# sergiud/SuiteSparse

Measured on AMD Instinct MI355X. Metric: GFLOP/s supernodal Cholesky factor (Common->fl / t_factorize), higher is better.
Workload: dtype f64; 1 GPU; poisson3d_200^3_geometricND_leaf4; n=8000000, nsuper=428821, parallelism=1 GPU

## Files before the change

include/cholmod_hip.h:

```cpp
#ifndef CHOLMOD_HIP_H
#define CHOLMOD_HIP_H

#include <stddef.h>
#include <stdint.h>

#ifdef __cplusplus
extern "C" {
#endif

#define CHOLMOD_HIP_OK            0
#define CHOLMOD_HIP_NOT_POSDEF    1
#define CHOLMOD_HIP_NO_DEVICE   (-1)
#define CHOLMOD_HIP_OUT_OF_MEMORY (-2)
#define CHOLMOD_HIP_TOO_LARGE   (-3)
#define CHOLMOD_HIP_INVALID     (-4)
#define CHOLMOD_HIP_GPU_PROBLEM (-5)

#define CHOLMOD_HIP_PLAN_DEFAULT   0
#define CHOLMOD_HIP_TILE128         4
#define CHOLMOD_HIP_NO_SMALL_FRONTS 16
#define CHOLMOD_HIP_NO_XCD_SWIZZLE 32
#define CHOLMOD_HIP_FIXED_OB       64
#define CHOLMOD_HIP_WIDE_OB       128
#define CHOLMOD_HIP_NO_CB_ASSIGN   2048
#define CHOLMOD_HIP_NO_FUSED_POTRF 512
#define CHOLMOD_HIP_NO_FUSED_TRSM 1024
#define CHOLMOD_HIP_NO_LEAF_PAIRS 4096
#define CHOLMOD_HIP_NO_EXCHANGE_LOOKAHEAD 256
#define CHOLMOD_HIP_CHAIN256     8192
#define CHOLMOD_HIP_PHI_TWIN    16384
#define CHOLMOD_HIP_CX_STORAGE   32768
#define CHOLMOD_HIP_FUSED_CB_EA   65536
#define CHOLMOD_HIP_PLAN_HOST_ONLY 2

typedef struct cholmod_hip_plan cholmod_hip_plan ;

int cholmod_hip_probe (void) ;

int cholmod_hip_memorysize (size_t *total_mem, size_t *available_mem) ;

int cholmod_hip_set_device (int device) ;
int cholmod_hip_device_count (int *count) ;

cholmod_hip_plan *cholmod_hip_plan_create (int64_t n, int64_t nsuper,
    const int64_t *super, const int64_t *pi, const int64_t *px,
    const int64_t *s, int flags, int *status) ;

void cholmod_hip_plan_destroy (cholmod_hip_plan *plan) ;

cholmod_hip_plan *cholmod_hip_plan_create_reach (int64_t n, int64_t nsuper,
    const int64_t *super, const int64_t *pi, const int64_t *px,
    const int64_t *s, int flags, const int64_t *reach_p, const int32_t *reach_first, int *status) ;

typedef int (*cholmod_hip_allreduce_fn) (void *dev_ptr, int64_t count_doubles,
    int group_first, int group_size, void *user) ;
cholmod_hip_plan *cholmod_hip_plan_create_dist (int64_t n, int64_t nsuper,
    const int64_t *super, const int64_t *pi, const int64_t *px,
    const int64_t *s, int flags, int rank, int world, int *status) ;
int cholmod_hip_set_allreduce (cholmod_hip_plan *plan,
    cholmod_hip_allreduce_fn fn, void *user) ;
int cholmod_hip_rccl_unique_id (void *id128) ;
int cholmod_hip_rccl_attach (cholmod_hip_plan *plan, const void *id128) ;
int cholmod_hip_rccl_detach (cholmod_hip_plan *plan) ;
int64_t cholmod_hip_debug_routing (cholmod_hip_plan *plan, int64_t cap, int64_t *pair_d, int64_t *pair_a,
    int64_t *cb_lo, int64_t *cb_hi) ;
int cholmod_hip_debug_schedule_hash (cholmod_hip_plan *plan, uint64_t *out16) ;
int64_t cholmod_hip_debug_cb_extend_add (cholmod_hip_plan *plan, int64_t cap, int64_t *out) ;
int64_t cholmod_hip_debug_fused_pair (cholmod_hip_plan *plan, int64_t pair, int64_t *desc, int32_t *inv, int32_t *rel) ;
int cholmod_hip_progress_enable (cholmod_hip_plan *plan, int enable) ;
int cholmod_hip_progress (cholmod_hip_plan *plan, int64_t *out12) ;
int64_t cholmod_hip_get_batches (cholmod_hip_plan *plan, int64_t *batch_of, int64_t *global_arena) ;
int cholmod_hip_get_partition (cholmod_hip_plan *plan, int64_t *owner) ;
int cholmod_hip_get_groups (cholmod_hip_plan *plan, int64_t *first, int64_t *size) ;
int cholmod_hip_gather_factor (cholmod_hip_plan *plan) ;

int cholmod_hip_factorize (cholmod_hip_plan *plan, const int64_t *Sp,
    const int64_t *Si, const int64_t *Snz, const double *Sx, double beta,
    int quick_return_if_not_posdef, double *Lx_host, int64_t *minor) ;

int cholmod_hip_upload_matrix (cholmod_hip_plan *plan, const int64_t *Sp,
    const int64_t *Si, const int64_t *Snz, const double *Sx) ;
int cholmod_hip_factorize_resident (cholmod_hip_plan *plan, double beta,
    int quick_return_if_not_posdef, int64_t *minor) ;

int cholmod_hip_set_value_map (cholmod_hip_plan *plan, const int64_t *src, int64_t snz,
    int64_t nvalues) ;
int cholmod_hip_values_begin (cholmod_hip_plan *plan, double **buffer, const int64_t **index,
    int64_t *count, int64_t *chunk_len) ;
int cholmod_hip_values_push_chunk (cholmod_hip_plan *plan, int64_t chunk) ;

int cholmod_hip_factorize_values_device (cholmod_hip_plan *plan, const double *dvalues, int64_t nvalues,
// ... 79 lines not shown
```

suitesparse_amd/cholmod.py:

```python
from __future__ import annotations

import ctypes as C
import os
import subprocess

import numpy as np

_HERE = os.path.dirname(os.path.abspath(__file__))
LIB_PATH = os.environ.get("CHOLMOD_AMD_LIB") or os.path.join(_HERE, "lib", "libcholmod_amd.so")
HOOKS_LIB_PATH = os.path.join(_HERE, "lib", "libcholmod_amd_testhooks.so")
CSRC = os.path.join(_HERE, "csrc")

CHOLMOD_MAXMETHODS = 9
CHOLMOD_HIP_NSTATS = 41

PATTERN, REAL, COMPLEX, ZOMPLEX = 0, 1, 2, 3
OK, NOT_INSTALLED, OUT_OF_MEMORY, TOO_LARGE, INVALID, GPU_PROBLEM = 0, -1, -2, -3, -4, -5
NOT_POSDEF = 1
NATURAL, GIVEN, POSTORDERED = 0, 1, 6
SIMPLICIAL, AUTO, SUPERNODAL = 0, 1, 2
SYS_A, SYS_LDLt, SYS_LD, SYS_DLt, SYS_L, SYS_Lt, SYS_D, SYS_P, SYS_Pt = range(9)
HIP_PLAN_HOST_ONLY = 2
HIP_WIDE_OB, HIP_NO_FUSED_POTRF, HIP_NO_FUSED_TRSM, HIP_PHI_TWIN = 128, 512, 1024, 16384
HIP_NO_SMALL_FRONTS = 16
HIP_FUSED_CB_EA = 65536
HIP_OK = 0
HIP_INVALID = -4
HIP_NO_DEVICE = -1


class Method(C.Structure):
    _fields_ = [("lnz", C.c_double), ("fl", C.c_double), ("ordering", C.c_int)]


ERRFUNC = C.CFUNCTYPE(None, C.c_int, C.c_char_p, C.c_int, C.c_char_p)
ALLREDUCE_FN = C.CFUNCTYPE(C.c_int, C.c_void_p, C.c_int64, C.c_int, C.c_int, C.c_void_p)


class Common(C.Structure):
    _fields_ = [
        ("supernodal", C.c_int), ("supernodal_switch", C.c_double),
        ("final_asis", C.c_int), ("final_super", C.c_int), ("final_ll", C.c_int),
        ("final_pack", C.c_int), ("final_monotonic", C.c_int), ("final_resymbol", C.c_int),
        ("zrelax", C.c_double * 3), ("nrelax", C.c_size_t * 3),
        ("prefer_upper", C.c_int), ("quick_return_if_not_posdef", C.c_int),
        ("print", C.c_int), ("nmethods", C.c_int), ("current", C.c_int), ("selected", C.c_int),
        ("method", Method * (CHOLMOD_MAXMETHODS + 1)),
        ("postorder", C.c_int), ("try_catch", C.c_int),
# ... 95 lines not shown
    "cholmod_l_hip_aat_values_grad_device", "cholmod_l_hip_aat_logdet_grad_device",
    "cholmod_l_hip_factor_grad_device", "cholmod_l_hip_factor_outer_grad_device", "cholmod_l_hip_factor_grad_to_host",
]
HIP_SYMBOLS = [
    "cholmod_hip_probe", "cholmod_hip_memorysize", "cholmod_hip_set_device", "cholmod_hip_device_count",
    "cholmod_hip_plan_create", "cholmod_hip_plan_destroy", "cholmod_hip_factorize",
    "cholmod_hip_plan_create_dist", "cholmod_hip_plan_create_reach", "cholmod_hip_set_allreduce", "cholmod_hip_get_partition",
    "cholmod_hip_get_groups", "cholmod_hip_get_batches", "cholmod_hip_progress_enable", "cholmod_hip_progress", "cholmod_hip_debug_schedule_hash", "cholmod_hip_diag_minmax", "cholmod_hip_values_begin", "cholmod_hip_values_push_chunk", "cholmod_hip_debug_routing",
    "cholmod_hip_gather_factor",
    "cholmod_hip_upload_matrix", "cholmod_hip_factorize_resident",
    "cholmod_hip_set_value_map",
    "cholmod_hip_factorize_values_device", "cholmod_hip_set_product_map", "cholmod_hip_download_matrix_values",
    "cholmod_hip_download_factor", "cholmod_hip_download_even_columns", "cholmod_hip_upload_factor", "cholmod_hip_solve",
    "cholmod_hip_set_perm", "cholmod_hip_solve_device", "cholmod_hip_residual_device", "cholmod_hip_refine_device",
    "cholmod_hip_get_maps", "cholmod_hip_get_stats", "cholmod_hip_set_profiling",
    "cholmod_hip_selinv_device", "cholmod_hip_selinv_gather_device", "cholmod_hip_selinv_download",
    "cholmod_hip_selinv_release", "cholmod_hip_selinv_info",
    "cholmod_hip_schur_device", "cholmod_hip_trailing_multiply_device",
    "cholmod_hip_factor_grad_device", "cholmod_hip_factor_outer_grad_device", "cholmod_hip_factor_grad_gather_device",
    "cholmod_hip_factor_grad_download", "cholmod_hip_factor_grad_release", "cholmod_hip_factor_grad_info",
    "cholmod_hip_values_grad_device", "cholmod_hip_logdet_device",
    "cholmod_hip_product_values_grad_device", "cholmod_hip_product_logdet_grad_device",
    "cholmod_hip_dense_partial_factor", "cholmod_hip_factor_checks", "cholmod_hip_factor_checks_local", "cholmod_hip_get_launch_profile", "cholmod_hip_debug_thin_cycles", "cholmod_hip_debug_launch_regions",
    "cholmod_hip_debug_cb_extend_add", "cholmod_hip_debug_fused_pair",
    "cholmod_hip_rccl_unique_id", "cholmod_hip_rccl_attach", "cholmod_hip_rccl_detach",
    "cholmod_hip_version",
]

PROBES_PATH = os.path.join(_HERE, "lib", "libcholmod_amd_probes.so")
PROBE_SYMBOLS = [
    "cholmod_hip_bench_update_kernel", "cholmod_hip_bench_update_pair", "cholmod_hip_bench_mfma_peak", "cholmod_hip_bench_mfma_peak2",
    "cholmod_hip_bench_mixed", "cholmod_hip_debug_potrf_cycles", "cholmod_hip_debug_panel_cycles",
    "cholmod_hip_debug_latency", "cholmod_hip_bench_mfma_ceiling", "cholmod_hip_probe_cu_mask", "cholmod_hip_probe_overlap", "cholmod_hip_debug_update_diff", "cholmod_hip_debug_diag_cycles", "cholmod_hip_bench_handoff",
]

_probes = None


def build(force: bool = False) -> str:
    if force:
        subprocess.check_call(["make", "-C", CSRC, "-s", "clean"])
    subprocess.check_call(["make", "-C", CSRC, "-s", "-j3"])
    return LIB_PATH


_libs = {}

# ... 129 lines not shown
    sig("cholmod_hip_factor_grad_release", C.c_int, [vp])
    sig("cholmod_hip_factor_grad_info", C.c_int, [vp, vp])
    sig("cholmod_l_hip_factor_grad_device", C.c_int, [sp, fc, vp, vp, vp, vp, cm])
    sig("cholmod_l_hip_factor_outer_grad_device", C.c_int, [sp, fc, dbl, vp, sz, vp, sz, sz, vp, vp, vp, cm])
    sig("cholmod_l_hip_factor_grad_to_host", C.c_int, [fc, vp, cm])
    sig("cholmod_hip_values_grad_device", C.c_int, [vp, C.c_int, dbl, vp, i64, vp, i64, i64, vp, i64, vp])
    sig("cholmod_hip_logdet_device", C.c_int, [vp, vp, vp])
    sig("cholmod_l_hip_values_grad_device", C.c_int, [sp, fc, dbl, vp, sz, vp, sz, sz, vp, vp, cm])
    sig("cholmod_l_hip_logdet_device", C.c_int, [fc, vp, vp, cm])
    sig("cholmod_hip_product_values_grad_device", C.c_int, [vp, C.c_int, dbl, vp, i64, vp, i64, i64, vp, vp, i64, vp])
    sig("cholmod_hip_product_logdet_grad_device", C.c_int, [vp, vp, vp, i64, vp])
    sig("cholmod_l_hip_aat_values_grad_device", C.c_int, [sp, fc, dbl, vp, sz, vp, sz, sz, vp, vp, vp, cm])
    sig("cholmod_l_hip_aat_logdet_grad_device", C.c_int, [sp, fc, vp, vp, vp, cm])
    sig("cholmod_hip_get_maps", C.c_int, [vp, vp, vp, vp])
    sig("cholmod_hip_get_stats", C.c_int, [vp, vp])
    sig("cholmod_hip_set_profiling", C.c_int, [vp, C.c_int])
    sig("cholmod_hip_dense_partial_factor", C.c_int, [vp, i64, i64, C.c_int, C.POINTER(i64)])
    sig("cholmod_hip_factor_checks", C.c_int, [vp, vp])
    sig("cholmod_hip_factor_checks_local", C.c_int, [vp, vp])
    sig("cholmod_hip_get_launch_profile", i64, [vp, i64, vp, vp, vp, vp, vp, vp])
    sig("cholmod_hip_debug_thin_cycles", C.c_int, [vp, i64, vp])
    sig("cholmod_hip_debug_launch_regions", i64, [vp, i64, i64, vp])
    sig("cholmod_hip_debug_cb_extend_add", i64, [vp, i64, vp])
    sig("cholmod_hip_debug_fused_pair", i64, [vp, i64, vp, vp, vp])
    sig("cholmod_hip_rccl_unique_id", C.c_int, [vp])
    sig("cholmod_hip_rccl_attach", C.c_int, [vp, vp])
    sig("cholmod_hip_rccl_detach", C.c_int, [vp])
    sig("cholmod_hip_version", C.c_char_p, [])
    _libs[path] = L
    return L


def probes():
    global _probes
    if _probes is not None:
        return _probes
    if not os.path.exists(PROBES_PATH):
        raise RuntimeError(f"{PROBES_PATH} is missing: build it with __graft_entry__.build()")
    L = C.CDLL(PROBES_PATH)
    vp, i64, dbl = C.c_void_p, C.c_int64, C.c_double
    for name, res, args in (
            ("cholmod_hip_bench_update_kernel", dbl, [i64, i64, i64, C.c_int, C.c_int]),
            ("cholmod_hip_bench_update_pair", dbl, [i64, i64, i64, i64, i64, C.c_int, C.c_int]),
            ("cholmod_hip_bench_mfma_peak", dbl, [C.c_int, C.c_int]),
            ("cholmod_hip_bench_mfma_peak2", dbl, [C.c_int, C.c_int, C.c_int, C.c_int]),
            ("cholmod_hip_bench_mixed", dbl, [C.c_int, C.c_int, C.c_int]),
# ... 606 lines not shown
```

suitesparse_amd/csrc/hip/engine.hip:

```cpp
#include "update_launch.hip.h"
#include "chain256_kernels.hip.h"
#include "exchange_internal.hip.h"
#include <thread>

namespace {

static void drop_product_map (cholmod_hip_plan *P)
{
    for (void *d : {(void *) P->d_pm_cp, (void *) P->d_pm_ia, (void *) P->d_pm_ib, (void *) P->d_pm_order}) if (d) (void) hipFree (d) ;
    P->d_pm_cp = P->d_pm_ia = P->d_pm_ib = nullptr ; P->d_pm_order = nullptr ;
    P->pm_set = false ; P->pm_na = 0 ;
    for (void *d : {(void *) P->d_pt_ptr, (void *) P->d_pt_c, (void *) P->d_pt_partner, (void *) P->d_pt_order, (void *) P->d_pt_gvals})
        if (d) (void) hipFree (d) ;
    P->d_pt_ptr = nullptr ; P->d_pt_c = P->d_pt_partner = P->d_pt_order = nullptr ; P->d_pt_gvals = nullptr ;
    P->pt_built = false ;
}

static void free_device (cholmod_hip_plan *P)
{
    drop_product_map (P) ;
    selinv_free (P) ;
    grad_free (P) ;
    for (hipEvent_t e : {P->fv_ev_in, P->fv_ev_out}) if (e) (void) hipEventDestroy (e) ;
    P->fv_ev_in = P->fv_ev_out = nullptr ;
// ... 1357 lines not shown

int64_t cholmod_hip_debug_fused_pair (cholmod_hip_plan *P, int64_t pair, int64_t *desc, int32_t *inv, int32_t *rel)
{
    if (!P) return CHOLMOD_HIP_INVALID ;
    const Schedule &S = P->sch ;
    const i64 np = (i64) S.ivp.size () ;
    if (pair < 0 || pair >= np || !desc) return np ;
    const InvPair &R = S.ivp [pair] ;
    i64 launch = -1 ;
    for (size_t z = 0 ; z < S.fz.size () && launch < 0 ; z++)
    {
        if (S.fz [z].front != R.parent) continue ;
        const size_t q = (size_t) (std::find (S.gfz.begin (), S.gfz.end (), (i32) z) - S.gfz.begin ()) ;
        for (size_t l = 0 ; l < S.launches.size () ; l++)
            if (S.launches [l].kind == K_UPD_W && q >= S.launches [l].goff && q < S.launches [l].goff + S.launches [l].ng) launch = (i64) l ;
    }
    const i64 d [8] = {R.parent, R.child, R.pnscol, R.pncb, R.nc, P->fr [R.child].cbp, R.mcb, launch} ;
    for (int t = 0 ; t < 8 ; t++) desc [t] = d [t] ;
    if (inv && P->d_invmap) HIPCHK (hipMemcpy (inv, P->d_invmap + R.inv, (size_t) R.pncb * sizeof (i32), hipMemcpyDeviceToHost)) ;
    if (rel && P->d_relmap) HIPCHK (hipMemcpy (rel, P->d_relmap + R.rel, (size_t) R.nc * sizeof (i32), hipMemcpyDeviceToHost)) ;
    return np ;
}

int64_t cholmod_hip_debug_launch_regions (cholmod_hip_plan *P, int64_t launch, int64_t cap, int64_t *out)
{
    if (!P || launch < 0 || launch >= (i64) P->sch.launches.size ()) return CHOLMOD_HIP_INVALID ;
    const Launch &L = P->sch.launches [launch] ;
    if (L.kind != K_UPD_W && L.kind != K_UPD_SMALL && L.kind != K_UPD_BIG && L.kind != K_UPD_PF) return 0 ;
    for (i64 q = 0 ; q < L.ng && q < cap ; q++)
    {
        const GemmGroup &G = P->sch.gg [L.goff + q] ;
        const i64 v [12] = {G.m, G.n, G.k, G.tri, G.c_in_cb, G.lda, G.ldc, G.ntiles, G.nblk, G.front, G.assign, G.swz} ;
        for (int t = 0 ; t < 12 ; t++) out [12 * q + t] = v [t] ;
    }
    return L.ng ;
}

int cholmod_hip_set_profiling (cholmod_hip_plan *P, int on)
{
    if (!P) return CHOLMOD_HIP_INVALID ;
    P->profiling = on != 0 ;
    return CHOLMOD_HIP_OK ;
}

int cholmod_hip_dense_partial_factor (double *F, int64_t nsrow, int64_t nscol, int flags,
    int64_t *info_out)
{
    if (!F || nsrow <= 0 || nscol <= 0 || nscol > nsrow) return CHOLMOD_HIP_INVALID ;
    if (!cholmod_hip_probe ()) return CHOLMOD_HIP_NO_DEVICE ;
    FrontD f ;
    memset (&f, 0, sizeof (f)) ;
    f.nscol = (i32) nscol ; f.nsrow = (i32) nsrow ; f.ncb = (i32) (nsrow - nscol) ; f.parent = -1 ;
    std::vector<FrontD> fr (1, f) ;
    Schedule S ;
// ... 58 lines not shown
```

suitesparse_amd/csrc/hip/plan.hip.h:

```cpp
#pragma once
#include "descriptors.hip.h"
#include "../../../include/cholmod_hip.h"

#include <rccl/rccl.h>

#include <algorithm>
#include <atomic>
#include <cmath>
#include <cstdio>
#include <cstdlib>
#include <cstring>
#include <map>
#include <functional>
#include <memory>
#include <new>
#include <queue>
#include <vector>
#include <atomic>
#include <chrono>

#ifdef CHOLMOD_HIP_TEST_HOOKS
#define TEST_ENV(name) getenv (name)
#else
#define TEST_ENV(name) ((const char *) nullptr)
// ... 211 lines not shown
    std::vector<SolveTask> sv_tasks ;
    std::vector<i32> sv_ptr ;
    std::vector<std::vector<i32>> sv_big ;
    SolveTask *d_sv = nullptr ;
    std::vector<InvTask> inv_tasks ;
    std::vector<i64> inv_first ;
    InvTask *d_inv_tasks = nullptr ;
    double *d_winv = nullptr ;
    bool winv_valid = false ;
    double *d_solved = nullptr ; i64 solved_cap = 0 ;
    double *d_sv_acc = nullptr ; i64 sv_acc_cap = 0 ;
    struct SbLaunch { i32 level, first, ntasks, grid ; } ;
    std::vector<SolveBlk> sb_tasks, sb_commit ;
    std::vector<SbLaunch> sb_launch, sb_commit_launch ;
    std::vector<i32> sb_lvl_ptr ;
    SolveBlk *d_sb_tasks = nullptr, *d_sb_commit = nullptr ;
    int sb_max_tasks = 0 ;
    long long *d_thin_tim = nullptr ;
    CheckTask *d_chk = nullptr ; i64 nchk = 0 ;
    double *d_chk_out = nullptr ;
    Schedule sch ;
    double exec_flops = 0 ;
    std::vector<i64> reach_p ;
    std::vector<i32> reach_first, head ;
    bool head_gather = true ;
    GatherGroup *d_xg = nullptr ; i32 *d_gmap = nullptr ;
    FuseD *d_fz = nullptr ; i32 *d_gfz = nullptr, *d_invmap = nullptr ;
    hipStream_t stream = nullptr ;
    hipStream_t stream2 = nullptr ;
    std::vector<hipEvent_t> sync_ev ;
    i64 *d_Ls = nullptr ;
    FrontD *d_fr = nullptr ;
    i32 *d_supermap = nullptr, *d_child = nullptr, *d_relmap = nullptr, *d_info = nullptr ;
    i32 *d_lvl_list = nullptr ;
    double *d_Lx = nullptr, *d_cb = nullptr ;
    ZeroGroup *d_zg = nullptr ; EaGroup *d_eg = nullptr ; PfGroup *d_pg = nullptr ;
    TrGroup *d_tg = nullptr ; GemmGroup *d_gg = nullptr ; i32 *d_sm = nullptr ;
    DgGroup *d_dg = nullptr ; RsGroup *d_rg = nullptr ; double *d_dinv = nullptr ;
    std::vector<i64> lpx ;
    i64 lx_local = 0 ;
    std::vector<i64> win_off ;
    i64 lx_fronts = 0 ;
    std::vector<i64> crel ;
    std::vector<RelPair> relpairs ;
    i64 relsize_all = 0 ;
    bool passthru = false ;
    i64 *d_crel = nullptr ; RelPair *d_relpairs = nullptr ;
// ... 45 lines not shown
    int factor_state = 0 ;
    hipEvent_t sc_ev_in = nullptr, sc_ev_out = nullptr ;
    struct Grad *gr = nullptr ;
    bool gr_index_valid = false ;
    volatile long long prog_fact = 0, prog_launch = 0, prog_xchg_enq = 0 ;
    long long *prog_dev = nullptr ;
    bool profiling = false ;
    double stats [CHOLMOD_HIP_NSTATS] = {0} ;
    double solve_seconds = 0 ;
    std::vector<float> launch_ms ;
    hipEvent_t ev0 = nullptr, ev1 = nullptr ;
    std::vector<hipEvent_t> evpool ;
} ;

static inline double *whole_factor (cholmod_hip_plan *P) { return P->world == 1 ? P->d_Lx : (P->full_valid ? P->d_Lx_full : nullptr) ; }
static inline const FrontD *whole_fronts (cholmod_hip_plan *P) { return P->world == 1 ? P->d_fr : P->d_fr_full ; }

void selinv_free (cholmod_hip_plan *P) ;
void selinv_gather_logdet_grad (cholmod_hip_plan *P, const i32 *colof, double *out, hipStream_t st) ;
void grad_free (cholmod_hip_plan *P) ;

namespace sship {

struct HeadInfo { const i32 *head ; const i64 *reach_p ; const i32 *first ; bool gather ; } ;

int build_host (cholmod_hip_plan *P) ;
void schedule_dense (const std::vector<FrontD> &fr, const i32 *ids, int nf,
    Schedule &S, int flags, const i32 *owner, const i32 *grp0, const i32 *grpn, int rank, int world,
    const char *assign_cb = nullptr, const i64 *win = nullptr, const i32 *child = nullptr, bool allow_half = false,
    const HeadInfo *heads = nullptr, const i64 *crel = nullptr, const std::vector<i64> *Ls = nullptr) ;

}
```

suitesparse_amd/csrc/hip/plan_build.hip:

```cpp
#include "plan.hip.h"

namespace sship {
namespace {

struct PlanBuilder
{
    cholmod_hip_plan *P ;
    const i64 n, nsuper ;
    int nlev = 0 ;
    std::vector<i32> cptr, call ;
    std::vector<double> wsub ;
    std::vector<i32> st_stack ;
    bool distribute = false, passthru = false, cx_storage = false ;
    int ownw = 128 ;
    std::vector<i64> cb_len_all ;
    std::vector<std::vector<i32>> rel_list ;
    std::vector<std::vector<i32>> batches ;

    explicit PlanBuilder (cholmod_hip_plan *P_) : P (P_), n (P_->n), nsuper (P_->nsuper) {}

    bool mine (i64 s) const { return P->rank >= P->grp0 [s] && P->rank < P->grp0 [s] + P->grpn [s] ; }
    template <typename F> void for_subtree (i32 root, F &&fn)
    {
        st_stack.clear () ;
// ... 617 lines not shown
    }
    void schedule_batches ()
    {
        Schedule &S = P->sch ;
        std::vector<i32> mine_ids, gen ;
        P->batch_launch0.clear () ;
        for (const auto &bt : batches)
        {
            P->batch_launch0.push_back (S.launches.size ()) ;
            mine_ids.clear () ; gen.clear () ;
            for (i32 sf : bt) if (mine (sf)) mine_ids.push_back (sf) ;
            if (mine_ids.empty ()) continue ;
            schedule_thin (mine_ids, gen) ;
            const i32 *ids = gen.data () ;
            const int nf = (int) gen.size () ;
            if (nf == 0) continue ;
            schedule_zero (ids, nf) ;
            const size_t ea0 = S.launches.size (), fz0 = S.fz.size (), ivp0 = S.ivp.size () ;
            schedule_extend_add (ids, nf, 0) ;
            const bool has_ea0 = S.launches.size () > ea0 ;
            schedule_dense (P->fr, ids, nf, S, P->flags, P->owner.data (), P->grp0.data (), P->grpn.data (),
                P->rank, P->world, P->assign_cb.data (), P->win_off.data (), P->child.data (),
                P->world == 1 && !P->force_shared,
                P->head.empty () ? nullptr : &heads, P->crel.data (), &P->Ls) ;
            if (S.fz.size () == fz0) { schedule_extend_add (ids, nf, 1) ; continue ; }
            std::vector<char> fused (nf, 0) ;
            {
                std::map<i32, int> at ;
                for (int q = 0 ; q < nf ; q++) at [ids [q]] = q ;
                for (size_t z = fz0 ; z < S.fz.size () ; z++) fused [at [S.fz [z].front]] = 1 ;
            }
            if (has_ea0)
                for (size_t z = ivp0 ; z < S.ivp.size () ; z++)
                    S.launches [ea0].bytes -= 24.0 * ((double) S.ivp [z].mcb * (S.ivp [z].mcb + 1) / 2) ;
            schedule_extend_add (ids, nf, 1, &fused) ;
        }
    }

    HeadInfo heads {nullptr, nullptr, nullptr, true} ;
    void choose_heads ()
    {
        P->head.clear () ;
        if (P->reach_p.empty () || P->world != 1 || P->force_shared || getenv ("CHOLMOD_HIP_NO_HEADS")) return ;
        if (P->flags & (CHOLMOD_HIP_PHI_TWIN | CHOLMOD_HIP_CX_STORAGE | CHOLMOD_HIP_TILE128)) return ;
        const ObThresholds obt = outer_block_thresholds () ;
        const bool all = getenv ("CHOLMOD_HIP_HEAD_ALL") && atoi (getenv ("CHOLMOD_HIP_HEAD_ALL")) != 0 ;
        auto rate = [] (int K) { return 1e12 * (K < 512 ? 60.0 : K < 1024 ? 70.0 : K < 2048 ? 74.5 : 75.0) ; } ;
        auto tri = [] (double m) { return m * (m + 1) / 2 ; } ;
        std::vector<i32> head (P->nsuper, 0) ;
        bool any = false ;
        for (i64 s = 0 ; s < P->nsuper ; s++)
        {
            const FrontD &f = P->fr [s] ;
            if (P->reach_p [s + 1] - P->reach_p [s] != f.nsrow || P->owner [s] < 0) continue ;
            const i32 *first = P->reach_first.data () + P->reach_p [s] ;
            const int OB = front_ob (f, P->flags, obt) ;
            double best = all ? 0.0 : 0.25e-3 ;
            for (int H = 256 ; H < std::min (OB, (int) f.nscol) ; H += 256)
            {
                i64 R = 0 ;
                for (int p = H ; p < f.nsrow ; p++) R += first [p] < H ;
                const double N = f.nsrow - H ;
                const double gain = all ? 2.0 * H * (tri (N) - tri ((double) R))
                    : 2.0 * H * tri (N) / rate (OB) - 2.0 * H * tri ((double) R) / rate (H) - 16.0 * tri (N) / 4e12 ;
                if (gain > best) { best = gain ; head [s] = H ; any = true ; }
            }
        }
        if (!any) return ;
        P->head.swap (head) ;
        P->head_gather = !getenv ("CHOLMOD_HIP_HEAD_NO_GATHER") ;
        heads = HeadInfo {P->head.data (), P->reach_p.data (), P->reach_first.data (), P->head_gather} ;
    }

    int run ()
    {
        int rc = init_fronts () ;
        if (rc != CHOLMOD_HIP_OK) return rc ;
        rc = build_etree () ;
        if (rc != CHOLMOD_HIP_OK) return rc ;
        assign_ownership () ;
        choose_heads () ;
        layout_local_factor () ;
        build_child_lists () ;
        choose_batches () ;
        rc = build_solve_tasks () ;
        if (rc != CHOLMOD_HIP_OK) return rc ;
        layout_windows () ;
        schedule_batches () ;
        for (const Launch &L : P->sch.launches) P->stats [40] += L.skipped ;
        return CHOLMOD_HIP_OK ;
    }
} ;

}
// ... 9 lines not shown
```

suitesparse_amd/csrc/hip/schedule_dense.hip:

```cpp
#include "plan.hip.h"

namespace sship {
namespace {

struct Upd { int q, kc, kk, t0, t1 ; bool cb, wide ; } ;

struct DenseScheduler
{
    const std::vector<FrontD> &fr ;
    const i32 *ids ; const int nf ;
    Schedule &S ;
    const int flags ;
    const i32 *owner, *grp0, *grpn ;
    const int rank, world ;
    const char *assign_cb ;
    const i64 *win ;
    const i32 *child ;
    const bool allow_half ;
    const HeadInfo *heads ;
    const i64 *crel ;
    const std::vector<i64> *Ls ;
    bool cx, twin, use_big ;
    ObThresholds obt ;
    int maxnscol = 0, maxrows = 0 ;
// ... 40 lines not shown
        by_launch = true ;
        { const char *e = getenv ("CHOLMOD_HIP_UPD3_HALF_MAX") ; w_half_max = e ? (i64) atoll (e) : (i64) 10240 ; }
        w_half_min = 512 ; w_min_k = 256 ; unfuse_tiles = w_min_tiles ;
        if (!allow_half || w_min_tiles <= 0) w_half_max = 0 ;
        if (w_half_max <= 0 || w_half_min > w_min_tiles) w_half_min = w_min_tiles ;
        one_region = false ;
        swz16 = false ;
        xla = !(flags & CHOLMOD_HIP_NO_EXCHANGE_LOOKAHEAD) ;
        balance_cb = !use_big && !getenv ("CHOLMOD_HIP_NO_CB_BALANCE") ;
        early.assign (nf, -1) ; early_open.assign (nf, -1) ; pf_done.assign (nf, -1) ;
        fuse_ea = (flags & CHOLMOD_HIP_FUSED_CB_EA) && world == 1 && allow_half && !twin && !use_big && w_min_tiles > 0
            && assign_cb && child && crel && Ls ;
        choose_chain () ;
    }

    i64 co (int c, i64 ld) const { return cx ? (i64) (c >> 1) * ld : (i64) c * ld ; }
    void twin_operands (GemmGroup &G, int origin, int kc) const
    {
        if ((origin | kc | G.k | G.m | G.n | G.lda | G.ldc) & 1) { fprintf (stderr, "cholmod_hip: twin plan with an odd region\n") ; abort () ; }
        if (!cx) G.lda *= 2 ;
        G.k /= 2 ;
    }
    int ob_of (const FrontD &f) const { return front_ob (f, flags, obt) ; }
    int head_of (int fid) const { return heads && heads->head ? heads->head [fid] : 0 ; }
    void ob_bounds (int q, int i0, int &o0, int &o1) const
    {
        const FrontD &f = fr [ids [q]] ;
        const int OBq = ob_of (f), H = head_of (ids [q]) ;
        if (H > 0 && i0 < H) o0 = 0 ;
        else if (H > 0) o0 = H + ((i0 - H) / OBq) * OBq ;
        else o0 = (i0 / OBq) * OBq ;
        o1 = std::min (o0 + (H > 0 && i0 < H ? H : OBq), (int) f.nscol) ;
    }
    bool is_shared (int fid) const { return owner && owner [fid] < 0 ; }
    bool windowed (int fid) const { return win && win [fid] >= 0 ; }
    i64 psx_at (int fid, int col) const
    {
        const FrontD &f = fr [fid] ;
        if (!windowed (fid)) return f.psx ;
        int OBq = ob_of (f), ob = col / OBq ;
        return win [fid] + (i64) (ob & 1) * window_len (f, OBq) - (i64) ob * OBq * f.nsrow ;
    }
    static i64 region_tiles (const GemmGroup &G)
    {
        i64 mt = (G.m + SMALL - 1) / SMALL, nt = (G.n + SMALL - 1) / SMALL ;
        return G.tri ? nt * (nt + 1) / 2 + (mt - nt) * nt : mt * nt ;
    }
    static i64 tri_tiles (int rows, int cols)
    {
        i64 mt = (rows + SMALL - 1) / SMALL, nt = (cols + SMALL - 1) / SMALL ;
        return nt * (nt + 1) / 2 + (mt - nt) * nt ;
    }
    XchgD xchg_of (int q, int c0) const
    {
        const FrontD &f = fr [ids [q]] ;
// ... 232 lines not shown
    void flush_updates ()
    {
        if (w_min_tiles > 0 && !use_big)
        {
            i64 pooled = 0 ;
            if (by_launch) for (auto &G : small) if (G.k >= w_min_k || region_tiles (G) >= w_min_tiles) pooled += region_tiles (G) ;
            std::vector<GemmGroup> keep ;
            for (auto &G : small)
            {
                const bool w = region_tiles (G) >= w_min_tiles || (by_launch && pooled >= w_half_min && G.k >= w_min_k) ;
                if (w) wav.push_back (G) ; else keep.push_back (G) ;
            }
            small.swap (keep) ;
        }
        flush_kind (big, K_UPD_BIG) ;
        flush_kind (small, K_UPD_SMALL) ;
        flush_kind (pfv, K_UPD_PF) ;
        flush_kind (wav, K_UPD_W) ;
        flush_gathered () ;
        carrier.clear () ;
    }
    void add_head_gathered (const Upd &x)
    {
        const int fid = ids [x.q], H = x.kk ;
        const FrontD &f = fr [fid] ;
        const i32 *first = heads->first + heads->reach_p [fid] ;
        auto tri_elems = [] (double m, double n) { return n * (n + 1) / 2 + (m - n) * n ; } ;
        double full = tri_elems (f.nsrow - H, f.nscol - H) + tri_elems (f.ncb, f.ncb), done = 0 ;
        auto gathered = [&] (int from, int ncols, bool to_cb)
        {
            const size_t m0 = S.gmap.size () ;
            int n = 0 ;
            for (int p = from ; p < f.nsrow ; p += 2)
            {
                if (first [p] >= H && (p + 1 >= f.nsrow || first [p + 1] >= H)) continue ;
                S.gmap.push_back (p) ; n += p < from + ncols ;
                if (p + 1 < f.nsrow) { S.gmap.push_back (p + 1) ; n += p + 1 < from + ncols ; }
            }
            const int m = (int) (S.gmap.size () - m0) ;
            if (n == 0) { S.gmap.resize (m0) ; return ; }
            GatherGroup X ;
            memset (&X, 0, sizeof (X)) ;
            X.g = blank_region (fid) ;
            X.g.a_off = X.g.b_off = f.psx ; X.g.lda = f.nsrow ;
            if (to_cb) { X.g.c_off = f.cb - f.nscol - (i64) f.nscol * f.ncb ; X.g.ldc = f.ncb ; X.g.c_in_cb = 1 ; }
            else { X.g.c_off = f.psx ; X.g.ldc = f.nsrow ; }
            X.g.m = m ; X.g.n = n ; X.g.k = H ; X.g.tri = 1 ;
            X.g.assign = (to_cb && assign_cb && assign_cb [fid]) ? 1 : 0 ;
            X.map = (i64) m0 ;
            done += tri_elems (m, n) ;
            gav.push_back (X) ;
        } ;
        if (x.t1 > x.t0) gathered (H, f.nscol - H, false) ;
        if (f.ncb > 0)
        {
            if (assign_cb && assign_cb [fid])
            {
                Launch Lz {K_ZERO, 0, 0, S.zg.size (), 0, 0} ;
                S.zg.push_back (ZeroGroup {f.cb, (i64) f.ncb, 0, 0}) ;
                Lz.ng = 1 ; Lz.grid = (f.ncb + ZERO_COLS - 1) / ZERO_COLS ;
                Lz.bytes = 8.0 * (double) f.ncb * (f.ncb + 1) / 2 ;
                S.launches.push_back (Lz) ;
            }
            gathered (f.nscol, f.ncb, true) ;
        }
        gav_skipped += 2.0 * H * std::max (0.0, full - done) ;
    }
    void flush_gathered ()
    {
        if (gav.empty ()) return ;
        Launch L {K_UPD_G, 0, 0, S.xg.size (), 0, 0} ;
        i64 tiles = 0 ;
        for (GatherGroup &X : gav)
        {
            GemmGroup &G = X.g ;
            const i64 mine = place_region (G, SMALL, true, tiles) ;
            G.nblk = (i32) mine ;
            G.tile_start = X.tile_start = (i32) tiles ;
            tiles += mine ;
            const double elems = (double) G.n * (G.n + 1) / 2 + (double) (G.m - G.n) * G.n ;
            L.flops += 2.0 * elems * G.k ;
            L.aux = std::max (L.aux, (int) G.k) ;
            L.bytes += (G.assign ? 8.0 : 16.0) * elems + 8.0 * ((double) G.m + G.n) * G.k ;
            S.xg.push_back (X) ;
        }
        L.ng = (int) (S.xg.size () - L.goff) ;
        L.grid = (int) tiles ;
        L.half = tiles < w_half_max ? 1 : 0 ;
        L.skipped = gav_skipped ;
        S.launches.push_back (L) ;
        gav.clear () ;
        gav_skipped = 0 ;
    }
// ... 155 lines not shown
    }
    void emit_step ()
    {
        for (const Upd &x : step) if (x.cb && is_shared (ids [x.q])) { join_far_gathers () ; break ; }
        const int ev_next = emit_next_columns_first () ;
        const bool any_next = ev_next != -2 ;
        const bool ff_unfuse_wide_k = unfuse_wide_k () ;
        for (const Upd &x : step)
        {
            const FrontD &f = fr [ids [x.q]] ;
            const int fid = ids [x.q] ;
            int c0 = x.t0 ;
            bool ahead = any_next && x.wide && is_shared (fid) && x.t1 > x.t0 ;
            if (ahead) c0 = std::min (x.t0 + MB, x.t1) ;
            bool ff = fuse_potrf && !(x.wide && is_shared (fid)) && !x.cb && c0 == x.t0 && f.nscol - x.t0 >= NB && x.t1 - c0 >= NB ;
            if (ff && w_min_tiles > 0 && !use_big && !is_shared (fid))
            {
                if (tri_tiles (f.nsrow - c0, x.t1 - c0) >= unfuse_tiles) ff = false ;
                if (ff_unfuse_wide_k && x.kk >= 512) ff = false ;
            }
            if (ff) pf_done [x.q] = x.t0 ;
            if (!x.wide && is_shared (fid) && x.t1 > c0) { add_chunk_update (x, c0, ff) ; continue ; }
            if (x.wide && is_shared (fid) && !x.cb) { if (x.t1 > c0) add_wide_shared (x, c0, x.t1) ; continue ; }
            if (x.cb && x.kc == 0 && x.kk == head_of (fid) && heads->gather) { add_head_gathered (x) ; continue ; }
            if (x.cb && windowed (fid)) { if (x.t1 > c0) add_outer_slabs (f, fid, x.kc, x.kk, c0, x.t1) ; }
            else if (x.t1 > c0) add_update (f, fid, c0, x.kc, x.kk, f.nsrow - c0, x.t1 - c0, false, x.wide, ff) ;
            if (x.cb && f.cbd) add_distributed_cb (x) ;
            else if (x.cb)
            {
                size_t nsm = small.size () ;
                add_update (f, fid, f.nscol, x.kc, x.kk, f.ncb, f.ncb, true, x.wide) ;
                if (fuse_ea && small.size () > nsm && x.kc == head_of (fid) && assign_cb [fid] && f.child_end > f.child_begin
                    && !is_shared (fid) && !windowed (fid))
                    carrier [fid] = small.back ().a_off ;
                if (windowed (fid) && f.own_g > 1 && balance_cb && small.size () > nsm) balance_cb_tiles (x) ;
            }
        }
        flush_updates () ;
        if (any_next)
            for (const Upd &x : step)
            {
                if (!x.wide || !is_shared (ids [x.q]) || x.t1 <= x.t0) continue ;
                if (x.cb && windowed (ids [x.q]))
                {
                    emit_win (x.q, 0, x.t0, std::min (x.t0 + MB, x.t1), 1, ev_next) ;
                    early_open [x.q] = x.t0 ;
                }
// ... 192 lines not shown
            }
        }
        Lt.ng = (int) (S.tg.size () - Lt.goff) ; Lt.grid = blocks ;
        if (Lt.ng) S.launches.push_back (Lt) ;
    }
    void run_chain64 ()
    {
        for (int i0 = 0 ; i0 < maxnscol ; i0 += NB)
        {
            enter_block_column (i0) ;
            emit_potrf (i0) ;
            std::vector<char> fused (nf, 0) ;
            emit_trsm_upd (i0, fused) ;
            emit_trsm (i0, fused) ;
            leave_sub_block (i0, NB) ;
            push_doubling_steps (i0, NB, &fused) ;
        }
    }

    void run ()
    {
        if (chain256) run_chain256 () ; else run_chain64 () ;
        join_far_gathers () ;
    }
} ;

}

void schedule_dense (const std::vector<FrontD> &fr, const i32 *ids, int nf,
    Schedule &S, int flags, const i32 *owner, const i32 *grp0, const i32 *grpn, int rank, int world,
    const char *assign_cb, const i64 *win, const i32 *child, bool allow_half, const HeadInfo *heads,
    const i64 *crel, const std::vector<i64> *Ls)
{
    DenseScheduler D (fr, ids, nf, S, flags, owner, grp0, grpn, rank, world, assign_cb, win, child, allow_half, heads, crel, Ls) ;
    D.run () ;
}

}
```

suitesparse_amd/csrc/host/numeric.c:

```c
#include "host_internal.h"
#ifdef _OPENMP
#include <omp.h>
#else
static int omp_get_thread_num (void) { return 0 ; }
#endif
#include <time.h>


int cholmod_l_gpu_memorysize (size_t *total_mem, size_t *available_mem, cholmod_common *Common)
{
    if (total_mem) *total_mem = 0 ;
    if (available_mem) *available_mem = 0 ;
    if (!Common) return 1 ;
    return cholmod_hip_memorysize (total_mem, available_mem) ;
}

int cholmod_l_gpu_probe (cholmod_common *Common)
{
    if (!Common) return 0 ;
    if (!cholmod_hip_probe ()) return 0 ;
    size_t t = 0, a = 0 ;
    if (cholmod_hip_memorysize (&t, &a) == 0) Common->gpuMemorySize = a ;
    return 1 ;
}
// ... 47 lines not shown

int ssamd_factor_has_cholesky_sizes (const cholmod_factor *L)
{
    if (!L || !L->is_super || !L->px || !L->super || !L->pi) return FALSE ;
    const Int *px = L->px ;
    if (L->nsuper > 0 && px [0] == 123456) return FALSE ;
    return (size_t) px [L->nsuper] <= L->xsize ;
}

static int plan_flags_of (const cholmod_factor *L, const cholmod_common *Common)
{
    int flags = Common->hip_flags ;
    if (L->hip_is_twin == 2) flags |= CHOLMOD_HIP_CX_STORAGE ;
    else if (L->hip_is_twin)
    {
        const char *e = getenv ("CHOLMOD_HIP_TWIN_FULL_K") ;
        if (!(e && atoi (e) != 0)) flags |= CHOLMOD_HIP_PHI_TWIN ;
    }
    return flags ;
}

static int engine_flags_of (const cholmod_factor *L, const cholmod_common *Common)
{
    const char *e = getenv ("CHOLMOD_HIP_NO_FUSED_CB_EA") ;
    if (L->hip_is_twin || Common->hip_world > 1 || (e && atoi (e) != 0)) return 0 ;
    return CHOLMOD_HIP_FUSED_CB_EA ;
}

static int ensure_plan_with (cholmod_factor *L, cholmod_common *Common, const int64_t *reach_p, const int32_t *reach_first) ;
int ssamd_ensure_plan (cholmod_factor *L, cholmod_common *Common) { return ensure_plan_with (L, Common, NULL, NULL) ; }

static int ensure_plan_with (cholmod_factor *L, cholmod_common *Common, const int64_t *reach_p, const int32_t *reach_first)
{
    if (!ssamd_factor_has_cholesky_sizes (L))
    { ERROR (CHOLMOD_INVALID, "L was analysed for SPQR (no Cholesky sizes)") ; return FALSE ; }
    int st = 0 ;
    int world = Common->hip_world > 1 ? Common->hip_world : 1 ;
    const int flags = plan_flags_of (L, Common) ;
    if (L->hip_plan && L->hip_plan_ahead && !L->hip_on_device && (L->hip_plan_ahead - 1 != flags || world > 1))
    {
        cholmod_hip_plan_destroy ((cholmod_hip_plan *) L->hip_plan) ;
        L->hip_plan = NULL ;
    }
    L->hip_plan_ahead = 0 ;
    if (L->hip_plan) return TRUE ;
    const double t_plan = omp_get_wtime () ;
    cholmod_hip_plan *P = (reach_p && world == 1)
        ? cholmod_hip_plan_create_reach ((int64_t) L->n, (int64_t) L->nsuper, L->super, L->pi, L->px, L->s,
            flags | engine_flags_of (L, Common), reach_p, reach_first, &st)
// ... 1111 lines not shown
```

Baseline: 64560 GFLOP/s.

## Add multi-level head stairs to skip structurally zero rows in front updates

Generalizes the single per-front head split into a sequence of stair boundaries (CSR head_p/head_v), chosen by a dynamic program over a cost model of gathered rank-K updates versus full outer-block updates. Each stair segment issues a gathered update that touches only rows whose reach starts before the boundary, with offsets adjusted for the column start. This aims to cut wasted GEMM/SYRK flops on zero-structured portions of large fronts. It is enabled by default through engine flags, adds planning cost and more gather launches, and relies on hardcoded throughput tables.

```diff
diff --git a/include/cholmod_hip.h b/include/cholmod_hip.h
--- a/include/cholmod_hip.h
+++ b/include/cholmod_hip.h
@@ -31,6 +31,7 @@
 #define CHOLMOD_HIP_PHI_TWIN    16384
 #define CHOLMOD_HIP_CX_STORAGE   32768
 #define CHOLMOD_HIP_FUSED_CB_EA   65536
+#define CHOLMOD_HIP_HEAD_STAIRS  131072
 #define CHOLMOD_HIP_PLAN_HOST_ONLY 2
 
 typedef struct cholmod_hip_plan cholmod_hip_plan ;
@@ -67,6 +68,7 @@
 int cholmod_hip_debug_schedule_hash (cholmod_hip_plan *plan, uint64_t *out16) ;
 int64_t cholmod_hip_debug_cb_extend_add (cholmod_hip_plan *plan, int64_t cap, int64_t *out) ;
 int64_t cholmod_hip_debug_fused_pair (cholmod_hip_plan *plan, int64_t pair, int64_t *desc, int32_t *inv, int32_t *rel) ;
+int64_t cholmod_hip_debug_head_stairs (cholmod_hip_plan *plan, int64_t *head_p, int64_t cap, int64_t *head_v) ;
 int cholmod_hip_progress_enable (cholmod_hip_plan *plan, int enable) ;
 int cholmod_hip_progress (cholmod_hip_plan *plan, int64_t *out12) ;
 int64_t cholmod_hip_get_batches (cholmod_hip_plan *plan, int64_t *batch_of, int64_t *global_arena) ;
diff --git a/suitesparse_amd/cholmod.py b/suitesparse_amd/cholmod.py
--- a/suitesparse_amd/cholmod.py
+++ b/suitesparse_amd/cholmod.py
@@ -24,6 +24,7 @@
 HIP_WIDE_OB, HIP_NO_FUSED_POTRF, HIP_NO_FUSED_TRSM, HIP_PHI_TWIN = 128, 512, 1024, 16384
 HIP_NO_SMALL_FRONTS = 16
 HIP_FUSED_CB_EA = 65536
+HIP_HEAD_STAIRS = 131072
 HIP_OK = 0
 HIP_INVALID = -4
 HIP_NO_DEVICE = -1
@@ -165,7 +166,7 @@
     "cholmod_hip_values_grad_device", "cholmod_hip_logdet_device",
     "cholmod_hip_product_values_grad_device", "cholmod_hip_product_logdet_grad_device",
     "cholmod_hip_dense_partial_factor", "cholmod_hip_factor_checks", "cholmod_hip_factor_checks_local", "cholmod_hip_get_launch_profile", "cholmod_hip_debug_thin_cycles", "cholmod_hip_debug_launch_regions",
-    "cholmod_hip_debug_cb_extend_add", "cholmod_hip_debug_fused_pair",
+    "cholmod_hip_debug_cb_extend_add", "cholmod_hip_debug_fused_pair", "cholmod_hip_debug_head_stairs",
     "cholmod_hip_rccl_unique_id", "cholmod_hip_rccl_attach", "cholmod_hip_rccl_detach",
     "cholmod_hip_version",
 ]
@@ -341,6 +342,7 @@
     sig("cholmod_hip_debug_thin_cycles", C.c_int, [vp, i64, vp])
     sig("cholmod_hip_debug_launch_regions", i64, [vp, i64, i64, vp])
     sig("cholmod_hip_debug_cb_extend_add", i64, [vp, i64, vp])
+    sig("cholmod_hip_debug_head_stairs", i64, [vp, vp, i64, vp])
     sig("cholmod_hip_debug_fused_pair", i64, [vp, i64, vp, vp, vp])
     sig("cholmod_hip_rccl_unique_id", C.c_int, [vp])
     sig("cholmod_hip_rccl_attach", C.c_int, [vp, vp])
diff --git a/suitesparse_amd/csrc/hip/engine.hip b/suitesparse_amd/csrc/hip/engine.hip
--- a/suitesparse_amd/csrc/hip/engine.hip
+++ b/suitesparse_amd/csrc/hip/engine.hip
@@ -1403,14 +1403,24 @@
     return np ;
 }
 
+int64_t cholmod_hip_debug_head_stairs (cholmod_hip_plan *P, int64_t *head_p, int64_t cap, int64_t *head_v)
+{
+    if (!P) return CHOLMOD_HIP_INVALID ;
+    const bool none = P->head_p.empty () ;
+    if (head_p) for (i64 s = 0 ; s <= P->nsuper ; s++) head_p [s] = none ? 0 : P->head_p [s] ;
+    const i64 nv = (i64) P->head_v.size () ;
+    if (head_v) for (i64 q = 0 ; q < nv && q < cap ; q++) head_v [q] = P->head_v [q] ;
+    return nv ;
+}
+
 int64_t cholmod_hip_debug_launch_regions (cholmod_hip_plan *P, int64_t launch, int64_t cap, int64_t *out)
 {
     if (!P || launch < 0 || launch >= (i64) P->sch.launches.size ()) return CHOLMOD_HIP_INVALID ;
     const Launch &L = P->sch.launches [launch] ;
-    if (L.kind != K_UPD_W && L.kind != K_UPD_SMALL && L.kind != K_UPD_BIG && L.kind != K_UPD_PF) return 0 ;
+    if (L.kind != K_UPD_W && L.kind != K_UPD_SMALL && L.kind != K_UPD_BIG && L.kind != K_UPD_PF && L.kind != K_UPD_G) return 0 ;
     for (i64 q = 0 ; q < L.ng && q < cap ; q++)
     {
-        const GemmGroup &G = P->sch.gg [L.goff + q] ;
+        const GemmGroup &G = L.kind == K_UPD_G ? P->sch.xg [L.goff + q].g : P->sch.gg [L.goff + q] ;
         const i64 v [12] = {G.m, G.n, G.k, G.tri, G.c_in_cb, G.lda, G.ldc, G.ntiles, G.nblk, G.front, G.assign, G.swz} ;
         for (int t = 0 ; t < 12 ; t++) out [12 * q + t] = v [t] ;
     }
diff --git a/suitesparse_amd/csrc/hip/plan.hip.h b/suitesparse_amd/csrc/hip/plan.hip.h
--- a/suitesparse_amd/csrc/hip/plan.hip.h
+++ b/suitesparse_amd/csrc/hip/plan.hip.h
@@ -257,7 +257,7 @@
     Schedule sch ;
     double exec_flops = 0 ;
     std::vector<i64> reach_p ;
-    std::vector<i32> reach_first, head ;
+    std::vector<i32> reach_first, head_p, head_v ;
     bool head_gather = true ;
     GatherGroup *d_xg = nullptr ; i32 *d_gmap = nullptr ;
     FuseD *d_fz = nullptr ; i32 *d_gfz = nullptr, *d_invmap = nullptr ;
@@ -349,7 +349,7 @@
 
 namespace sship {
 
-struct HeadInfo { const i32 *head ; const i64 *reach_p ; const i32 *first ; bool gather ; } ;
+struct HeadInfo { const i32 *head_p, *head_v ; const i64 *reach_p ; const i32 *first ; bool gather ; } ;
 
 int build_host (cholmod_hip_plan *P) ;
 void schedule_dense (const std::vector<FrontD> &fr, const i32 *ids, int nf,
diff --git a/suitesparse_amd/csrc/hip/plan_build.hip b/suitesparse_amd/csrc/hip/plan_build.hip
--- a/suitesparse_amd/csrc/hip/plan_build.hip
+++ b/suitesparse_amd/csrc/hip/plan_build.hip
@@ -663,7 +663,7 @@
             schedule_dense (P->fr, ids, nf, S, P->flags, P->owner.data (), P->grp0.data (), P->grpn.data (),
                 P->rank, P->world, P->assign_cb.data (), P->win_off.data (), P->child.data (),
                 P->world == 1 && !P->force_shared,
-                P->head.empty () ? nullptr : &heads, P->crel.data (), &P->Ls) ;
+                P->head_v.empty () ? nullptr : &heads, P->crel.data (), &P->Ls) ;
             if (S.fz.size () == fz0) { schedule_extend_add (ids, nf, 1) ; continue ; }
             std::vector<char> fused (nf, 0) ;
             {
@@ -678,25 +678,100 @@
         }
     }
 
-    HeadInfo heads {nullptr, nullptr, nullptr, true} ;
+    HeadInfo heads {nullptr, nullptr, nullptr, nullptr, true} ;
+    static double stair_rate (int K)
+    {
+        static const int NA = 8, kk [NA] = {256, 512, 768, 1024, 1536, 2048, 3072, 4096} ;
+        static const double tf [NA] = {47.0, 62.4, 67.5, 66.9, 69.7, 69.5, 73.2, 73.4} ;
+        if (K <= kk [0]) return 1e12 * tf [0] ;
+        for (int q = 1 ; q < NA ; q++)
+            if (K <= kk [q]) return 1e12 * (tf [q - 1] + (tf [q] - tf [q - 1]) * (double) (K - kk [q - 1]) / (double) (kk [q] - kk [q - 1])) ;
+        return 1e12 * tf [NA - 1] ;
+    }
+    static void choose_stairs (const FrontD &f, const i32 *first, int OB, bool all_levels, std::vector<i32> &out)
+    {
+        auto tri = [] (double m) { return m * (m + 1) / 2 ; } ;
+        const int lim = std::min ((int) f.nscol, 3 * OB), nb = lim > 0 ? (lim - 1) / 256 : 0, W = OB / 256 ;
+        if (nb < 1) return ;
+        if (all_levels)
+        {
+            for (int i = 1 ; i <= nb ; i++)
+            {
+                const int H = 256 * i ;
+                bool leaves = false ;
+                for (int p = H ; p < f.nsrow && !leaves ; p++) leaves = first [p] >= H ;
+                if (!leaves) break ;
+                out.push_back (H) ;
+            }
+            return ;
+        }
+        std::vector<double> R (nb + 1, 0.0), best (nb + 1, 0.0) ;
+        std::vector<int> prev (nb + 1, -1) ;
+        for (int i = 1 ; i <= nb ; i++)
+        {
+            i64 r = 0 ;
+            for (int p = 256 * i ; p < f.nsrow ; p++) r += first [p] < 256 * i ;
+            R [i] = (double) r ;
+        }
+        auto tail = [&] (int H)
+        {
+            double t = 0 ;
+            for (int a = H ; a < f.nscol ; a += OB)
+            {
+                const int b = std::min (a + OB, (int) f.nscol) ;
+                t += 2.0 * (b - a) * tri ((double) (f.nsrow - b)) / stair_rate (b - a) ;
+            }
+            return t ;
+        } ;
+        for (int i = 1 ; i <= nb ; i++)
+        {
+            const double N = f.nsrow - 256 * i ;
+            best [i] = 1e300 ;
+            for (int g = std::max (0, i - W) ; g < i ; g++)
+            {
+                const int K = 256 * (i - g) ;
+                const double t = best [g] + 2.0 * K * tri (R [i]) / stair_rate (K) + 16.0 * tri (N) / 4e12 + 0.1e-3 ;
+                if (t < best [i]) { best [i] = t ; prev [i] = g ; }
+            }
+        }
+        int last = 0 ;
+        double cost = tail (0) ;
+        for (int i = 1 ; i <= nb ; i++)
+        {
+            const double t = best [i] + tail (256 * i) ;
+            if (t < cost) { cost = t ; last = i ; }
+        }
+        const size_t o0 = out.size () ;
+        for (int i = last ; i > 0 ; i = prev [i]) out.push_back (256 * i) ;
+        std::reverse (out.begin () + o0, out.end ()) ;
+    }
     void choose_heads ()
     {
-        P->head.clear () ;
+        P->head_p.clear () ; P->head_v.clear () ;
         if (P->reach_p.empty () || P->world != 1 || P->force_shared || getenv ("CHOLMOD_HIP_NO_HEADS")) return ;
         if (P->flags & (CHOLMOD_HIP_PHI_TWIN | CHOLMOD_HIP_CX_STORAGE | CHOLMOD_HIP_TILE128)) return ;
         const ObThresholds obt = outer_block_thresholds () ;
         const bool all = getenv ("CHOLMOD_HIP_HEAD_ALL") && atoi (getenv ("CHOLMOD_HIP_HEAD_ALL")) != 0 ;
+        const bool stairs = (P->flags & CHOLMOD_HIP_HEAD_STAIRS) && !all ;
+        const bool stairs_all = stairs && getenv ("CHOLMOD_HIP_HEAD_STAIRS_ALL") && atoi (getenv ("CHOLMOD_HIP_HEAD_STAIRS_ALL")) != 0 ;
         auto rate = [] (int K) { return 1e12 * (K < 512 ? 60.0 : K < 1024 ? 70.0 : K < 2048 ? 74.5 : 75.0) ; } ;
         auto tri = [] (double m) { return m * (m + 1) / 2 ; } ;
-        std::vector<i32> head (P->nsuper, 0) ;
-        bool any = false ;
+        std::vector<i32> head_p (P->nsuper + 1, 0), head_v ;
         for (i64 s = 0 ; s < P->nsuper ; s++)
         {
+            head_p [s + 1] = head_p [s] ;
             const FrontD &f = P->fr [s] ;
             if (P->reach_p [s + 1] - P->reach_p [s] != f.nsrow || P->owner [s] < 0) continue ;
             const i32 *first = P->reach_first.data () + P->reach_p [s] ;
             const int OB = front_ob (f, P->flags, obt) ;
+            if (stairs)
+            {
+                choose_stairs (f, first, OB, stairs_all, head_v) ;
+                head_p [s + 1] = (i32) head_v.size () ;
+                continue ;
+            }
             double best = all ? 0.0 : 0.25e-3 ;
+            int head = 0 ;
             for (int H = 256 ; H < std::min (OB, (int) f.nscol) ; H += 256)
             {
                 i64 R = 0 ;
@@ -704,13 +779,14 @@
                 const double N = f.nsrow - H ;
                 const double gain = all ? 2.0 * H * (tri (N) - tri ((double) R))
                     : 2.0 * H * tri (N) / rate (OB) - 2.0 * H * tri ((double) R) / rate (H) - 16.0 * tri (N) / 4e12 ;
-                if (gain > best) { best = gain ; head [s] = H ; any = true ; }
-            }
-        }
-        if (!any) return ;
-        P->head.swap (head) ;
+                if (gain > best) { best = gain ; head = H ; }
+            }
+            if (head > 0) { head_v.push_back (head) ; head_p [s + 1] = (i32) head_v.size () ; }
+        }
+        if (head_v.empty ()) return ;
+        P->head_p.swap (head_p) ; P->head_v.swap (head_v) ;
         P->head_gather = !getenv ("CHOLMOD_HIP_HEAD_NO_GATHER") ;
-        heads = HeadInfo {P->head.data (), P->reach_p.data (), P->reach_first.data (), P->head_gather} ;
+        heads = HeadInfo {P->head_p.data (), P->head_v.data (), P->reach_p.data (), P->reach_first.data (), P->head_gather} ;
     }
 
     int run ()
diff --git a/suitesparse_amd/csrc/hip/schedule_dense.hip b/suitesparse_amd/csrc/hip/schedule_dense.hip
--- a/suitesparse_amd/csrc/hip/schedule_dense.hip
+++ b/suitesparse_amd/csrc/hip/schedule_dense.hip
@@ -86,15 +86,32 @@
         G.k /= 2 ;
     }
     int ob_of (const FrontD &f) const { return front_ob (f, flags, obt) ; }
-    int head_of (int fid) const { return heads && heads->head ? heads->head [fid] : 0 ; }
+    int stairs_of (int fid, const i32 *&h) const
+    {
+        if (!heads || !heads->head_p) return 0 ;
+        h = heads->head_v + heads->head_p [fid] ;
+        return heads->head_p [fid + 1] - heads->head_p [fid] ;
+    }
+    int head_of (int fid) const { const i32 *h ; const int k = stairs_of (fid, h) ; return k ? h [k - 1] : 0 ; }
+    bool ends_stair (int fid, int col) const
+    {
+        const i32 *h ;
+        const int k = stairs_of (fid, h) ;
+        return k && std::binary_search (h, h + k, (i32) col) ;
+    }
     void ob_bounds (int q, int i0, int &o0, int &o1) const
     {
         const FrontD &f = fr [ids [q]] ;
-        const int OBq = ob_of (f), H = head_of (ids [q]) ;
-        if (H > 0 && i0 < H) o0 = 0 ;
-        else if (H > 0) o0 = H + ((i0 - H) / OBq) * OBq ;
-        else o0 = (i0 / OBq) * OBq ;
-        o1 = std::min (o0 + (H > 0 && i0 < H ? H : OBq), (int) f.nscol) ;
+        const i32 *h ;
+        const int OBq = ob_of (f), k = stairs_of (ids [q], h), H = k ? h [k - 1] : 0 ;
+        if (i0 < H)
+        {
+            const int j = (int) (std::upper_bound (h, h + k, (i32) i0) - h) ;
+            o0 = j ? h [j - 1] : 0 ; o1 = h [j] ;
+            return ;
+        }
+        o0 = H + ((i0 - H) / OBq) * OBq ;
+        o1 = std::min (o0 + OBq, (int) f.nscol) ;
     }
     bool is_shared (int fid) const { return owner && owner [fid] < 0 ; }
     bool windowed (int fid) const { return win && win [fid] >= 0 ; }
@@ -373,7 +390,7 @@
     }
     void add_head_gathered (const Upd &x)
     {
-        const int fid = ids [x.q], H = x.kk ;
+        const int fid = ids [x.q], kc = x.kc, H = x.kc + x.kk ;
         const FrontD &f = fr [fid] ;
         const i32 *first = heads->first + heads->reach_p [fid] ;
         auto tri_elems = [] (double m, double n) { return n * (n + 1) / 2 + (m - n) * n ; } ;
@@ -393,11 +410,11 @@
             GatherGroup X ;
             memset (&X, 0, sizeof (X)) ;
             X.g = blank_region (fid) ;
-            X.g.a_off = X.g.b_off = f.psx ; X.g.lda = f.nsrow ;
+            X.g.a_off = X.g.b_off = f.psx + (i64) kc * f.nsrow ; X.g.lda = f.nsrow ;
             if (to_cb) { X.g.c_off = f.cb - f.nscol - (i64) f.nscol * f.ncb ; X.g.ldc = f.ncb ; X.g.c_in_cb = 1 ; }
             else { X.g.c_off = f.psx ; X.g.ldc = f.nsrow ; }
-            X.g.m = m ; X.g.n = n ; X.g.k = H ; X.g.tri = 1 ;
-            X.g.assign = (to_cb && assign_cb && assign_cb [fid]) ? 1 : 0 ;
+            X.g.m = m ; X.g.n = n ; X.g.k = x.kk ; X.g.tri = 1 ;
+            X.g.assign = (to_cb && kc == 0 && assign_cb && assign_cb [fid]) ? 1 : 0 ;
             X.map = (i64) m0 ;
             done += tri_elems (m, n) ;
             gav.push_back (X) ;
@@ -405,7 +422,7 @@
         if (x.t1 > x.t0) gathered (H, f.nscol - H, false) ;
         if (f.ncb > 0)
         {
-            if (assign_cb && assign_cb [fid])
+            if (kc == 0 && assign_cb && assign_cb [fid])
             {
                 Launch Lz {K_ZERO, 0, 0, S.zg.size (), 0, 0} ;
                 S.zg.push_back (ZeroGroup {f.cb, (i64) f.ncb, 0, 0}) ;
@@ -415,11 +432,17 @@
             }
             gathered (f.nscol, f.ncb, true) ;
         }
-        gav_skipped += 2.0 * H * std::max (0.0, full - done) ;
+        gav_skipped += 2.0 * x.kk * std::max (0.0, full - done) ;
+    }
+    void park_skipped ()
+    {
+        if (gav_skipped <= 0) return ;
+        for (auto it = S.launches.rbegin () ; it != S.launches.rend () ; ++it)
+            if (it->kind == K_UPD_G) { it->skipped += gav_skipped ; gav_skipped = 0 ; return ; }
     }
     void flush_gathered ()
     {
-        if (gav.empty ()) return ;
+        if (gav.empty ()) { park_skipped () ; return ; }
         Launch L {K_UPD_G, 0, 0, S.xg.size (), 0, 0} ;
         i64 tiles = 0 ;
         for (GatherGroup &X : gav)
@@ -621,7 +644,7 @@
             if (ff) pf_done [x.q] = x.t0 ;
             if (!x.wide && is_shared (fid) && x.t1 > c0) { add_chunk_update (x, c0, ff) ; continue ; }
             if (x.wide && is_shared (fid) && !x.cb) { if (x.t1 > c0) add_wide_shared (x, c0, x.t1) ; continue ; }
-            if (x.cb && x.kc == 0 && x.kk == head_of (fid) && heads->gather) { add_head_gathered (x) ; continue ; }
+            if (x.cb && ends_stair (fid, x.kc + x.kk) && heads->gather) { add_head_gathered (x) ; continue ; }
             if (x.cb && windowed (fid)) { if (x.t1 > c0) add_outer_slabs (f, fid, x.kc, x.kk, c0, x.t1) ; }
             else if (x.t1 > c0) add_update (f, fid, c0, x.kc, x.kk, f.nsrow - c0, x.t1 - c0, false, x.wide, ff) ;
             if (x.cb && f.cbd) add_distributed_cb (x) ;
@@ -860,6 +883,7 @@
     {
         if (chain256) run_chain256 () ; else run_chain64 () ;
         join_far_gathers () ;
+        park_skipped () ;
     }
 } ;
 
diff --git a/suitesparse_amd/csrc/host/numeric.c b/suitesparse_amd/csrc/host/numeric.c
--- a/suitesparse_amd/csrc/host/numeric.c
+++ b/suitesparse_amd/csrc/host/numeric.c
@@ -93,9 +93,9 @@
 
 static int engine_flags_of (const cholmod_factor *L, const cholmod_common *Common)
 {
-    const char *e = getenv ("CHOLMOD_HIP_NO_FUSED_CB_EA") ;
-    if (L->hip_is_twin || Common->hip_world > 1 || (e && atoi (e) != 0)) return 0 ;
-    return CHOLMOD_HIP_FUSED_CB_EA ;
+    const char *e = getenv ("CHOLMOD_HIP_NO_FUSED_CB_EA"), *h = getenv ("CHOLMOD_HIP_NO_HEAD_STAIRS") ;
+    if (L->hip_is_twin || Common->hip_world > 1) return 0 ;
+    return ((e && atoi (e) != 0) ? 0 : CHOLMOD_HIP_FUSED_CB_EA) | ((h && atoi (h) != 0) ? 0 : CHOLMOD_HIP_HEAD_STAIRS) ;
 }
 
 static int ensure_plan_with (cholmod_factor *L, cholmod_common *Common, const int64_t *reach_p, const int32_t *reach_first) ;
```

Result: no change. 64820 GFLOP/s, median of 6 (+0.4%).
